# SamArgt/AudioSourceSep

Measured on AMD Instinct MI355X. Metric: Glow fwd+logdet passes/sec on 64×64×1 mel tiles (K=32,L=3), 1→8 MI355X, higher is better.
Workload: dtype f16x3

## Files before the change

audiosourcesep_amd/csrc/glowk.hip:

```cpp
#include "glowk_engine.h"
#include "glowk_light.h"

namespace glowk_eng {
thread_local std::string g_err;
}
using namespace glowk_eng;

namespace glowk_eng {

}

namespace glowk_detail {
int num_cus() {
  static int n = 0;
  if (n == 0) {
    int dev = 0; hipDeviceProp_t prop;
    if (hipGetDevice(&dev) == hipSuccess && hipGetDeviceProperties(&prop, dev) == hipSuccess) n = prop.multiProcessorCount;
    if (n <= 0) n = 256;
  }
  return n;
}
void launch_fail(const std::string& m) { fail(m); }
static EnvSwitches read_env() {
  auto on = [](const char* n) { return getenv(n) != nullptr; };
  return EnvSwitches{on("GLOWK_BWD_LIGHT_4"), on("GLOWK_NO_FUSE"), on("GLOWK_WGRAD_PLAIN"), on("GLOWK_CO_OFF"), on("GLOWK_Q_OFF"), on("GLOWK_CO_TRAIN_OFF"),
                     on("GLOWK_TRAIN_RECOMPUTE"), on("GLOWK_TRAIN_PERSTEP"), on("GLOWK_PG_JOIN")};
}
static EnvSwitches g_env = read_env();
const EnvSwitches& env() { return g_env; }
void reload_env() { g_env = read_env(); }
#define GLOWK_EXTERN_NET(CI_, NF_) extern template NetLaunch launch_net_t<CI_, NF_>(const NetArgs&, NetCall, hipStream_t, bool);
GLOWK_NET_SHAPES(GLOWK_EXTERN_NET)
#undef GLOWK_EXTERN_NET
}

namespace glowk_eng {
using glowk_detail::num_cus;
using glowk_detail::launch_net_t;

NetCall net_call(const glowk_handle* h, int dir, bool store, bool split) {
  if (h->precision == GLOWK_PREC_F32 || !split) return NetCall{dir, NET_EXACT, store};
  return NetCall{dir, h->precision == GLOWK_PREC_F16X2 && dir == NET_FWD && !store ? NET_SPLIT2 : NET_SPLIT3, store};
}

int* flagp(const glowk_handle* h) { return h->precision == GLOWK_PREC_F32 ? nullptr : h->d_flag; }

float bwd_norm_target(float xlim_b) {
  if (!(xlim_b >= 0.125f)) return 0.0f;
  int e = 0;
  std::frexp(xlim_b * 0.5f, &e);
  return std::ldexp(1.0f, std::min(e - 1, 10));
}

NetLaunch launch_net_raw(int c, int F, const NetArgs& a, NetCall call, hipStream_t s, bool dry) {
#define NETCASE(CI_, NF_) if (c == 2 * CI_ && F == 32 * NF_) return launch_net_t<CI_, NF_>(a, call, s, dry);
  GLOWK_NET_SHAPES(NETCASE)
#undef NETCASE
  return glowk_detail::net_failed("unsupported (channels, n_filters) combination: c=" + std::to_string(c) + " F=" + std::to_string(F));
}

int launch_net(glowk_handle* h, int level, int c, int F, const NetArgs& a, hipStream_t s, NetCall call, NetLaunch* out = nullptr) {
  if (h->profiling) {
    while (h->ev_pool.size() < h->ev_used + 2) {
      OwnedEvent e;
      HIPCHK(event_create(e, hipEventDefault));
      h->ev_pool.push_back(std::move(e));
    }
    HIPCHK(hipEventRecord(h->ev_pool[h->ev_used], s));
  }
  const NetLaunch r = launch_net_raw(c, F, a, call, s);
  if (!r.failed) {
    ++h->family_launches[r.family];
    if (r.co) ++h->family_launches[FAM_CO];
    if (r.q) ++h->family_launches[FAM_Q];
  }
  if (h->profiling) {
    HIPCHK(hipEventRecord(h->ev_pool[h->ev_used + 1], s));
    h->ev_used += 2;
// ... 1143 lines not shown
```

audiosourcesep_amd/csrc/glowk_co.h:

```cpp
#pragma once
#include "glowk_kernels.h"

constexpr int CO_PX = 128;
constexpr int CO_PSTR = 132;

template <int KIN, int MOUT, int NF, int MODE>
struct RingC {
  static constexpr int MODE7 = net_dir<MODE>;
  using S = RingS<KIN, MOUT, NF, MODE7, 2>;
  static constexpr bool FUSE = (MODE & NET_FUSE) != 0;
  static constexpr bool SAVE = MODE7 == NET_FWD_SAVE, BWD = MODE7 == NET_BWD;
  static constexpr bool MERGE = S::NMT <= 3;
  static constexpr bool M0LAST = S::NMT % 3 == 2;
  static constexpr bool STORE = (MODE & NET_STORE) != 0;
  static constexpr int MODEX = net_dir<MODE> | (MODE & NET_STORE);
  static constexpr int NFH = S::NFH, NRB = S::NRB, NMT = S::NMT, KS = S::KS;
  static constexpr int UNITP = S::MAINP / 2;
  static constexpr int UNIT4 = S::MAIN4 / 2;
  static constexpr int PPW = UNITP / 4;
  static constexpr int NG = NFH / 2;
  static constexpr int K1PW = (S::K1P + 3) / 4;
  static constexpr int EPN = BWD ? 0 : S::EPN;
  static constexpr int MASKN = BWD ? 2 * 4 * NF * 64 : 0;
  static constexpr size_t LDS_BYTES = (size_t)3 * UNIT4 * 16 + (size_t)2 * S::K14 * 16 + (size_t)EPN * 4 + (size_t)MASKN * 2 +
                                      (FUSE ? (size_t)36 * CO_PSTR * 4 + CO_PX * 16 : 0);
  static constexpr bool FITS = (MODE7 == NET_FWD || MODE7 == NET_FWD2 || SAVE || BWD) && !(MODE & NET_HALF) && (!STORE || ((SAVE || BWD) && !FUSE)) && S::NGRP == 1 && (NMT == 2 || NMT == 3 || (NMT == 5 && !STORE && !BWD)) &&
                               (!FUSE || (MOUT == 36 && !BWD)) && KS <= 3 && NF % 4 == 0 && NFH >= 2 && NFH % 2 == 0 && UNITP % 4 == 0 && PPW == NG &&
                               2 * LDS_BYTES <= 160 * 1024 + 1;
  static constexpr int XST = STORE ? 8 : 0;
  static constexpr int z_acts(int z) { int n = 0; for (int t = z * NFH; t < (z + 1) * NFH; ++t) n += (t % NMT == 0) ? 1 : 0; return n; }
  static constexpr int z_st(int z) { return STORE ? z_acts(z) * (8 + (SAVE ? 1 : 0)) : 0; }
  __device__ static const float4* main_unit(const float4* img, int pass, int i, int half) { return S::main_chunk(img, pass, i) + (size_t)half * UNIT4; }
  __device__ static const float4* out_unit(const float4* img, int pass, int z) { return S::out_chunk(img, pass, 0) + (size_t)z * UNIT4; }
};

__device__ __forceinline__ void co_bar() {
  __builtin_amdgcn_s_waitcnt(0xC07F);
  h3_barrier();
}

template <int N>
__device__ __forceinline__ void co_end() {
  __builtin_amdgcn_s_waitcnt((N & 15) | 0x0070 | ((N >> 4) << 14));
  h3_barrier();
}
template <int N>
__device__ __forceinline__ void co_end_st(bool more) {
  if (more) co_end<N + 1>();
  else co_end<N>();
}

struct CoCtx {
  float4 *m0, *m1, *d;
  const float4* img;
  int w4;
  unsigned voff;
};

template <int NFH, int MODE7, int H, int TAG, int K1P>
__device__ __forceinline__ void co_Y(const float4* slot, const h8 (&bh)[2], const h8 (&bl)[2], f32x4 (&acc2)[2 * NFH][2], int lane,
                                     const float4* src, float4* dst, int w4, unsigned voff) {
  const h8* buf = reinterpret_cast<const h8*>(slot) + lane;
  const char* ub = uniform_ptr(src);
  constexpr int NG = NFH / 2;
  h8 A[2][4];
  auto load = [&](h8 (&d)[4], int gi) {
    d[0] = buf[((2 * gi) * 2 + 0) * 64];
    d[1] = buf[((2 * gi) * 2 + 1) * 64];
    d[2] = buf[((2 * gi + 1) * 2 + 0) * 64];
    d[3] = buf[((2 * gi + 1) * 2 + 1) * 64];
  };
  load(A[0], 0);
#pragma unroll
  for (int gi = 0; gi < NG; ++gi) {
    const int o0 = H * NFH + 2 * gi, o1 = o0 + 1;
    if (gi + 1 < NG) load(A[(gi + 1) & 1], gi + 1);
    if constexpr (H == 1) {
      const int piece = gi * 4 + w4;
// ... 102 lines not shown
}

template <int KIN, int MOUT, int NF, int MODE, int PASS, bool SOLO>
__device__ __forceinline__ void co_pass(const NetArgs& a, const H3Ctx& hc, const CoCtx& c, const float* epl, float* pl,
                                        const h8 (&xh)[(RingC<KIN, MOUT, NF, MODE>::KS)][2], const h8 (&xl)[(RingC<KIN, MOUT, NF, MODE>::KS)][2],
                                        const int (&q)[2], const bool (&qok)[2], int lane, int kq, f32x4 (&keep)[(RingC<KIN, MOUT, NF, MODE>::NMT)][2]) {
  using G = RingC<KIN, MOUT, NF, MODE>;
  using S = typename G::S;
  constexpr int NRB = G::NRB, NFH = G::NFH, MODE7 = G::MODE7;
  constexpr int f2base = PASS * NFH * 32;
  constexpr bool SECOND = !SOLO && PASS == 1;
  f32x4 acc2[NRB][2];
#pragma unroll
  for (int ob = 0; ob < NRB; ++ob)
#pragma unroll
    for (int r = 0; r < 4; ++r) {
      const float b = G::BWD ? 0.0f : epl[f2base + ob * 16 + 4 * kq + r];
      acc2[ob][0][r] = b;
      acc2[ob][1][r] = b;
    }
  const bool st = G::SAVE && PASS == 0 && hc.wok;
  constexpr int XST = PASS == 0 ? G::XST : 0;
  h8 bh[2], bl[2];
#pragma nounroll
  for (int i0 = 0; i0 < NF; i0 += 2) {
    if (i0 > 0 || (SECOND && !G::M0LAST)) stage4<G::UNITP, 73>(G::main_unit(c.img, PASS, i0, 1), c.m1, c.w4, c.voff);
    if constexpr (SECOND && G::M0LAST) {
      if (i0 == 0) stage4<G::UNITP, 77>(G::main_unit(c.img, PASS, 0, 0), c.m0, c.w4, c.voff);
    }
    h3s_X<KIN, MOUT, NF, G::MODEX, 2, 0, PASS, G::STORE>(a, hc, i0, xh, xl, lane, bh, bl);
    if (SECOND && G::M0LAST && i0 == 0) co_end<0>();
    else co_end_st<G::PPW + XST>(st);
    co_Y<NFH, MODE7, 0, 1, S::K1P>(c.m0, bh, bl, acc2, lane, hc.k1img + (size_t)((i0 + 2) % NF) * S::K14, hc.k1s0, c.w4, c.voff);
    co_end_st<G::K1PW + XST>(st);
    co_Y<NFH, MODE7, 1, 2, S::K1P>(c.m1, bh, bl, acc2, lane, G::main_unit(c.img, PASS, i0 + 1, 0), c.m0, c.w4, c.voff);
    co_bar();
    stage4<G::UNITP, 74>(G::main_unit(c.img, PASS, i0 + 1, 1), c.m1, c.w4, c.voff);
    h3s_X<KIN, MOUT, NF, G::MODEX, 2, 1, PASS, G::STORE>(a, hc, i0 + 1, xh, xl, lane, bh, bl);
    co_end_st<G::PPW + XST>(st);
    co_Y<NFH, MODE7, 0, 3, S::K1P>(c.m0, bh, bl, acc2, lane, hc.k1img + (size_t)((i0 + 3) % NF) * S::K14, hc.k1s1, c.w4, c.voff);
    co_end_st<G::K1PW + XST>(st);
    co_Y<NFH, MODE7, 1, 4, S::K1P>(c.m1, bh, bl, acc2, lane, i0 + 2 < NF ? G::main_unit(c.img, PASS, i0 + 2, 0) : G::out_unit(c.img, PASS, 1), c.m0,
                                   c.w4, c.voff);
    co_bar();
  }
  f32x4 acc3[G::NMT][2];
  co_Z<KIN, MOUT, NF, MODE, PASS, SOLO, 0>(a, hc, c, epl, pl, acc2, acc3, bh, bl, q, qok, lane, kq, keep);
  co_Z<KIN, MOUT, NF, MODE, PASS, SOLO, 1>(a, hc, c, epl, pl, acc2, acc3, bh, bl, q, qok, lane, kq, keep);
  if constexpr (G::NMT >= 3) co_Z<KIN, MOUT, NF, MODE, PASS, SOLO, 2>(a, hc, c, epl, pl, acc2, acc3, bh, bl, q, qok, lane, kq, keep);
  if constexpr (G::NMT >= 4) co_Z<KIN, MOUT, NF, MODE, PASS, SOLO, 3>(a, hc, c, epl, pl, acc2, acc3, bh, bl, q, qok, lane, kq, keep);
  if constexpr (G::NMT >= 5) co_Z<KIN, MOUT, NF, MODE, PASS, SOLO, 4>(a, hc, c, epl, pl, acc2, acc3, bh, bl, q, qok, lane, kq, keep);
}

template <int KIN, int MOUT, int NF, int MODE, bool SPLIT>
__global__ __launch_bounds__(256, 2) void k_net_h3c(NetArgs a) {
  using G = RingC<KIN, MOUT, NF, MODE>;
  using S = typename G::S;
  constexpr int KS = G::KS;
  constexpr int SGN = G::BWD ? -1 : 1;
  static_assert(G::FITS, "shape");
  static_assert(!(G::FUSE && SPLIT), "the fused coupling needs both passes in one workgroup");

  const int tid = threadIdx.x;
  __shared__ __attribute__((aligned(1024))) float4 slotM0[G::UNIT4];
  __shared__ __attribute__((aligned(1024))) float4 slotM1[G::UNIT4];
  __shared__ __attribute__((aligned(1024))) float4 slotD[G::UNIT4];
  __shared__ __attribute__((aligned(1024))) float4 k1slot0[S::K14];
  __shared__ __attribute__((aligned(1024))) float4 k1slot1[S::K14];
  float* epl = nullptr;
  if constexpr (!G::BWD) { __shared__ float epl_arr[S::EPN]; epl = epl_arr; }
  unsigned short* mkl = nullptr;
  if constexpr (G::BWD) { __shared__ __attribute__((aligned(1024))) unsigned short mkl_arr[G::MASKN]; mkl = mkl_arr; }
  float* plds = nullptr;
  float4* vstash = nullptr;
  if constexpr (G::FUSE) {
    __shared__ float plds_arr[36 * CO_PSTR];
    __shared__ float4 vstash_arr[CO_PX];
    plds = plds_arr; vstash = vstash_arr;
  }
  const int lane = tid & 63;
  const int wave = __builtin_amdgcn_readfirstlane(tid >> 6);
  const int n16 = lane & 15;
  const int kq = lane >> 4;
  const int qbase = ((int)blockIdx.x * 4 + wave) * 32;
  const int q[2] = {G::STORE ? qbase + 2 * n16 : qbase + n16, G::STORE ? qbase + 2 * n16 + 1 : qbase + 16 + n16};
  const bool qok[2] = {q[0] < a.Q, q[1] < a.Q};
  const int pass0 = SPLIT ? (int)blockIdx.y : 0;

  H3Ctx hc;
  hc.sA = hc.sB = hc.sD = nullptr; hc.k1s0 = k1slot0; hc.k1s1 = k1slot1;
  hc.k1img = a.RSp; hc.img = a.RSp; hc.mkl = mkl; hc.mk2off = 4 * NF * 64; hc.pl = plds;
  hc.wblk = (size_t)blockIdx.x * 4 + wave;
  hc.wok = (long)hc.wblk * 32 < a.Q;
  hc.w4 = wave; hc.voff = (unsigned)lane * 16u; hc.ub[0] = hc.ub[1] = 1.0f;
  CoCtx c;
  c.m0 = slotM0; c.m1 = slotM1; c.d = slotD; c.img = a.RSp; c.w4 = wave; c.voff = (unsigned)lane * 16u;

  stage4<G::UNITP, 60>(G::main_unit(c.img, pass0, 0, 0), slotM0, c.w4, c.voff);
  stage4<G::UNITP, 61>(G::main_unit(c.img, pass0, 0, 1), slotM1, c.w4, c.voff);
  stage4<G::UNITP, 62>(G::out_unit(c.img, pass0, 0), slotD, c.w4, c.voff);
  stage4<S::K1P, 63>(hc.k1img, k1slot0, c.w4, c.voff);
  stage4<S::K1P, 64>(hc.k1img + S::K14, k1slot1, c.w4, c.voff);
  if constexpr (G::BWD) {
    stage4<NF / 2, 65>(reinterpret_cast<const float4*>(a.mask1 + (size_t)blockIdx.x * 4 * NF * 64), reinterpret_cast<float4*>(mkl), c.w4, c.voff);
    stage4<NF / 2, 66>(reinterpret_cast<const float4*>(a.mask2 + (size_t)blockIdx.x * 4 * NF * 64), reinterpret_cast<float4*>(mkl + 4 * NF * 64), c.w4, c.voff);
  }

  h8 xh[KS][2], xl[KS][2];
  float xmax = 0.0f;
  {
    const int hw = a.h * a.w;
#pragma unroll
    for (int hf = 0; hf < 2; ++hf) {
      const int qq = qok[hf] ? q[hf] : 0;
      const int rem = qq % hw;
      const int i = rem / a.w, j0 = rem % a.w;
      const float* base = a.vin + (long)qq * a.in_stride + a.in_off;
      if constexpr (G::BWD) {
        float v[KS][8];
        float pm = 0.0f;
#pragma unroll
        for (int s = 0; s < KS; ++s) {
          gather8<KIN, false, SGN>(base, i, j0, a.h, a.w, a.in_stride, qok[hf], 32 * s + 8 * kq, v[s]);
          pm = range8(pm, v[s]);
        }
        pm = nan_max(pm, __shfl_xor(pm, 16, 64));
        pm = nan_max(pm, __shfl_xor(pm, 32, 64));
        xmax = nan_max(xmax, pm);
        const float fac = G::STORE ? 1.0f : pixel_norm(pm, a.bnorm, hc.ub[hf]);
#pragma unroll
        for (int s = 0; s < KS; ++s) {
#pragma unroll
          for (int j = 0; j < 8; ++j) v[s][j] *= fac;
          split8(v[s], xh[s][hf], xl[s][hf]);
        }
      } else if constexpr (S::STK) {
        xmax = gather_stacked<KIN, SGN, G::MODE7 == NET_FWD2, KS, S::KSX>(base, i, j0, a.h, a.w, a.in_stride, qok[hf], kq, xh, xl, hf, xmax);
      } else {
#pragma unroll
        for (int s = 0; s < KS; ++s) {
          float v[8];
          gather8<KIN, true, SGN>(base, i, j0, a.h, a.w, a.in_stride, qok[hf], 32 * s + 8 * kq, v);
          xmax = range8(xmax, v);
          split8(v, xh[s][hf], xl[s][hf]);
        }
      }
    }
  }
  if constexpr (G::FUSE) {
    if (tid < CO_PX) {
      const int qv = (int)blockIdx.x * CO_PX + tid;
      vstash[tid] = qv < a.Q ? *reinterpret_cast<const float4*>(a.vin + (size_t)qv * 4) : float4{0.f, 0.f, 0.f, 0.f};
    }
  }
  if constexpr (!G::BWD)
    for (int i = tid; i < S::EPN; i += 256) epl[i] = a.eph[i];
  if (((G::BWD && !G::STORE) ? !(xmax <= 3.0e38f) : !(xmax <= a.xlim)) && a.flag) *a.flag = 1;
  if (a.xmax_out) range_probe(a.xmax_out, xmax);
  asm volatile("s_waitcnt vmcnt(0)" ::: "memory");
  __syncthreads();

  f32x4 keep[G::NMT][2];
  if constexpr (SPLIT) {
    if (pass0 == 0) co_pass<KIN, MOUT, NF, MODE, 0, true>(a, hc, c, epl, plds, xh, xl, q, qok, lane, kq, keep);
    else co_pass<KIN, MOUT, NF, MODE, 1, true>(a, hc, c, epl, plds, xh, xl, q, qok, lane, kq, keep);
  } else {
    co_pass<KIN, MOUT, NF, MODE, 0, false>(a, hc, c, epl, plds, xh, xl, q, qok, lane, kq, keep);
    co_pass<KIN, MOUT, NF, MODE, 1, false>(a, hc, c, epl, plds, xh, xl, q, qok, lane, kq, keep);
  }
  if constexpr (G::FUSE) {
    __syncthreads();
    fused_couple<CO_PX, CO_PSTR>(a, plds, vstash, tid);
  }
}
```

audiosourcesep_amd/csrc/glowk_kernels.h:

```cpp
#pragma once
#include "glowk_act_scale.h"

#include <hip/hip_runtime.h>
#include <utility>
#include <stdint.h>

typedef float f32x16 __attribute__((ext_vector_type(16)));

#define GLOWK_GPTR(p) ((const __attribute__((address_space(1))) void*)(p))
#define GLOWK_LPTR(p) ((__attribute__((address_space(3))) void*)(p))

__device__ __forceinline__ int mfma_row(int r, int hh) { return (r & 3) + 8 * (r >> 2) + 4 * hh; }

struct NetArgs {
  const float* vin;
  int in_stride, in_off;
  int Q, h, w;
  const float* K1p;
  const float* ep;
  const float4* R0p;
  unsigned short* mask1;
  unsigned short* mask2;
  float* P;
  size_t pstride;
// ... 1186 lines not shown
                                         f32x4 (&acc3)[(RingS<KIN, MOUT, NF, MODE, NP>::G0N)][2], h8 (&bh)[2], h8 (&bl)[2], int g, const int (&q)[2],
                                         const bool (&qok)[2], int lane, int kq, f32x4 (&keep)[(RingS<KIN, MOUT, NF, MODE, NP>::G0N)][2],
                                         std::integer_sequence<int, Z...>) {
  (h3s_Z<KIN, MOUT, NF, MODE, NP, P0, PASS, SOLO, Z>(a, c, epl, acc2, acc3, bh, bl, g, q, qok, lane, kq, keep), ...);
}

template <int KIN, int MOUT, int NF, int MODE, int NP, int P0, int PASS, bool SOLO>
__device__ __forceinline__ void h3s_pass(const NetArgs& a, const H3Ctx& c, const float* epl, const h8 (&xh)[(RingS<KIN, MOUT, NF, MODE, NP>::KS)][2],
                                         const h8 (&xl)[(RingS<KIN, MOUT, NF, MODE, NP>::KS)][2], int g, const int (&q)[2], const bool (&qok)[2], int lane, int kq,
                                         f32x4 (&keep)[(RingS<KIN, MOUT, NF, MODE, NP>::G0N)][2]) {
  using G = RingS<KIN, MOUT, NF, MODE, NP>;
  constexpr int NRB = G::NRB;
  constexpr int f2base = PASS * G::NFH * 32;
  f32x4 acc2[NRB][2];
#pragma unroll
  for (int ob = 0; ob < NRB; ++ob)
#pragma unroll
    for (int r = 0; r < 4; ++r) {
      const float b = net_dir<MODE> == NET_BWD ? 0.0f : epl[f2base + ob * 16 + 4 * kq + r];
      acc2[ob][0][r] = b;
      acc2[ob][1][r] = b;
    }
  h8 bh[2], bl[2];
#pragma nounroll
  for (int i0 = 0; i0 < NF; i0 += 2) {
    h3s_X<KIN, MOUT, NF, MODE, NP, 0, PASS>(a, c, i0, xh, xl, lane, bh, bl);
    h3_x_end<MODE, PASS, 8 * G::PXH>(c);
    if (PASS >= 1 && !SOLO && G::NCH == 1 && i0 == 0 && !g)
      stage4<G::MAINP, 50>(G::out_chunk(c.img, PASS, 0), c.sD, c.w4, c.voff);
    h3s_Y<KIN, MOUT, NF, MODE, NP, 1>(P0 ? c.sB : c.sA, bh, bl, acc2, lane, g, true, G::main_chunk(c.img, PASS, i0 + 1), P0 ? c.sA : c.sB,
                         c.k1img + (size_t)((i0 + 2) % NF) * G::K14, c.k1s0, c.w4, c.voff);
    h3_barrier();
    h3s_X<KIN, MOUT, NF, MODE, NP, 1, PASS>(a, c, i0 + 1, xh, xl, lane, bh, bl);
    h3_x_end<MODE, PASS, 8 * G::PXH>(c);
    h3s_Y<KIN, MOUT, NF, MODE, NP, 2>(P0 ? c.sA : c.sB, bh, bl, acc2, lane, g, i0 + 2 < NF || G::NCH >= 2,
                         i0 + 2 < NF ? G::main_chunk(c.img, PASS, i0 + 2) : G::out_chunk(c.img, PASS, 1),
                         P0 ? c.sB : c.sA, c.k1img + (size_t)((i0 + 3) % NF) * G::K14, c.k1s1, c.w4, c.voff);
    h3_barrier();
  }
  f32x4 acc3[G::G0N][2];
  h3s_tail<KIN, MOUT, NF, MODE, NP, P0, PASS, SOLO>(a, c, epl, acc2, acc3, bh, bl, g, q, qok, lane, kq, keep, std::make_integer_sequence<int, 2 * G::NCH>());
}

template <int KIN, int MOUT, int NF, int MODE, int NP, int PASS, int P0>
__device__ __forceinline__ void h3s_passes(const NetArgs& a, const H3Ctx& c, const float* epl, const h8 (&xh)[(RingS<KIN, MOUT, NF, MODE, NP>::KS)][2],
                                           const h8 (&xl)[(RingS<KIN, MOUT, NF, MODE, NP>::KS)][2], int g, const int (&q)[2], const bool (&qok)[2], int lane, int kq,
                                           f32x4 (&keep)[(RingS<KIN, MOUT, NF, MODE, NP>::G0N)][2]) {
  h3s_pass<KIN, MOUT, NF, MODE, NP, P0, PASS, false>(a, c, epl, xh, xl, g, q, qok, lane, kq, keep);
  if constexpr (PASS + 1 < NP) h3s_passes<KIN, MOUT, NF, MODE, NP, PASS + 1, (RingS<KIN, MOUT, NF, MODE, NP>::NCH + 1 + P0) & 1>(a, c, epl, xh, xl, g, q, qok, lane, kq, keep);
}

__device__ __forceinline__ bool fz_not_finite(float v) { return !(fabsf(v) <= 3.0e38f); }

template <int PXW = 256, int PSTR = FUSE_PSTR>
__device__ __forceinline__ void fused_couple(const NetArgs& a, const float* pl, const float4* vst, int tid) {
  const int wave = tid >> 6, lane = tid & 63;
  const int px = wave * 32 + (lane & 31), k = lane >> 5;
  const int q = (int)blockIdx.x * PXW + px;
  const bool qok = q < a.Q;
  const int w = a.w, hw = a.h * a.w, nrows = PXW / w;
  const int pp = (qok ? q : 0) % hw;
  const int i = pp / w, j = pp % w, r = px / w;
  float ols = 0.0f, ot = 0.0f;
  bool missing = false;
#pragma unroll
  for (int tap = 0; tap < 9; ++tap) {
    const int dy = tap / 3 - 1, dx = tap % 3 - 1;
    const int ii = i + dy, jj = j + dx;
    if (ii < 0 || ii >= a.h || jj < 0 || jj >= w) continue;
    const int rr = r + dy;
    if (rr < 0 || rr >= nrows) { missing = true; continue; }
    const int spx = px + dy * w + dx;
    ols += pl[(tap * 4 + k) * PSTR + spx];
    ot += pl[(tap * 4 + 2 + k) * PSTR + spx];
  }
  ols += a.fz_b3[k];
  ot += a.fz_b3[2 + k];
  float lsum = 0.0f;
  const float4 v4 = vst[px];
  const float vk = k ? v4.y : v4.x;
  const float log_s = tanhf(ols);
  const float sc = expf(log_s);
  const float yk = a.fz_inverse ? (vk - ot) / sc : sc * vk + ot;
  const float yo = __shfl_xor(yk, 32, 64);
  const float y[4] = {k ? yo : yk, k ? yk : yo, v4.z, v4.w};
  if (qok && a.fz_osave) a.fz_osave[(size_t)q * 2 + k] = ols;
  if (qok && !missing) {
    lsum = log_s;
    bool bad = fz_not_finite(ols) | fz_not_finite(ot) | fz_not_finite(yk);
    if (bad && a.flag) *a.flag = 1;
    float z0, z1;
    if (a.fz_A) {
      z0 = a.fz_b[2 * k]; z1 = a.fz_b[2 * k + 1];
#pragma unroll
      for (int ci = 0; ci < 4; ++ci) {
        z0 = fmaf(y[ci], a.fz_A[ci * 4 + 2 * k], z0);
        z1 = fmaf(y[ci], a.fz_A[ci * 4 + 2 * k + 1], z1);
      }
    } else {
      z0 = y[2 * k]; z1 = y[2 * k + 1];
    }
    *reinterpret_cast<float2*>(a.fz_out + (size_t)q * a.fz_out_stride + a.fz_out_off + 2 * k) = float2{z0, z1};
  } else if (qok) {
    float* e = a.fz_edge + (((size_t)blockIdx.x * 4 + (r == 0 ? 0 : 1)) * FUSE_EW + j) * 4;
    e[k] = ols;
    e[2 + k] = ot;
  }
  for (int te = tid; te < 2 * w * 4; te += 2 * PXW) {
    const int which = te / (4 * w), jt = (te / 4) % w, ch = te & 3;
    float hsum = 0.0f;
#pragma unroll
    for (int dx = -1; dx <= 1; ++dx) {
      const int js = jt + dx;
      if (js < 0 || js >= w) continue;
      const int tap = (which ? 0 : 6) + dx + 1;
      hsum += pl[(tap * 4 + ch) * PSTR + (which ? (nrows - 1) * w : 0) + js];
    }
    a.fz_edge[(((size_t)blockIdx.x * 4 + 2 + which) * FUSE_EW + jt) * 4 + ch] = hsum;
  }
  if (a.fz_ldpart) {
    double d = (double)lsum;
#pragma unroll
    for (int o = 32; o > 0; o >>= 1) d += __shfl_down(d, o, 64);
    if (lane == 0) a.fz_ldpart[(size_t)blockIdx.x * (PXW / 32) + wave] = d;
  }
}

template <int KIN, int MOUT, int NF, int MODE, int NP, bool SPLIT>
__global__ __launch_bounds__(512, 2) void k_net_h3s(NetArgs a) {
  using G = RingS<KIN, MOUT, NF, MODE, NP>;
  constexpr int KS = G::KS;
  constexpr int SGN = (net_dir<MODE> == NET_BWD) ? -1 : 1;
  static_assert(G::FITS, "shape");

  __shared__ float4 slotA[G::MAIN4];
  __shared__ float4 slotB[G::MAIN4];
  __shared__ float4 slotD[G::MAIN4];
  __shared__ float4 k1slot0[G::K14];
  __shared__ float4 k1slot1[G::K14];
  __shared__ float epl[G::EPN];
  __shared__ __attribute__((aligned(16))) unsigned short mkl[G::MASK2B / 2 + 8];
  __shared__ float plds[G::FUSE ? 36 * FUSE_PSTR : 1];
  __shared__ float4 vstash[G::FUSE ? 256 : 1];
  static_assert(!G::FUSE || (G::MERGE && !SPLIT && MOUT == 36), "the fused coupling needs both passes in one workgroup and a 4-channel level");
  static_assert(!(MODE & NET_STORE) || G::PXH == 1, "hidden stores (training): half-wave form only -- with two pixel halves a wave whose second half lies "
                                            "beyond Q would issue fewer stores than h3_x_end's counted wait assumes");

  const int tid = threadIdx.x;
  const int lane = tid & 63;
  const int wave = __builtin_amdgcn_readfirstlane(tid >> 6);
  const int g = wave >> 2;
  const int n16 = lane & 15;
  const int kq = lane >> 4;
  const int qbase = (blockIdx.x * 8 + (tid >> 6)) * (16 * G::PXH);
  const int q[2] = {qbase + n16, G::PXH == 2 ? qbase + 16 + n16 : qbase + n16};
  const bool qok[2] = {q[0] < a.Q, G::PXH == 2 && q[1] < a.Q};

  H3Ctx c;
  c.sA = slotA; c.sB = slotB; c.sD = slotD; c.k1s0 = k1slot0; c.k1s1 = k1slot1;
  const int solo_pass = SPLIT ? (int)blockIdx.y : 0;
  c.k1img = a.RSp;
  c.img = a.RSp;
  c.mkl = mkl;
  c.mk2off = 8 * NF * 64;
  c.pl = plds;
  c.wblk = (size_t)blockIdx.x * 8 + wave;
  c.wok = (long)c.wblk * (16 * G::PXH) < a.Q;
  c.w4 = wave & 3;
  c.voff = (unsigned)lane * 16u;
  c.ub[0] = c.ub[1] = 1.0f;

  if (!g) {
    stage4<G::MAINP, 60>(G::main_chunk(c.img, solo_pass, 0), slotA, c.w4, c.voff);
    stage4<G::MAINP, 61>(G::out_chunk(c.img, solo_pass, 0), slotD, c.w4, c.voff);
    if (net_dir<MODE> == NET_BWD)
      stage4<NF, 64>(reinterpret_cast<const float4*>(a.mask1 + (size_t)blockIdx.x * 8 * NF * 64), reinterpret_cast<float4*>(mkl), c.w4, c.voff);
  } else {
    stage4<G::K1P, 62>(c.k1img, k1slot0, c.w4, c.voff);
// ... 78 lines not shown
```

audiosourcesep_amd/csrc/glowk_launch.h:

```cpp
#pragma once
#include "glowk_kernels.h"
#include "glowk_co.h"
#include "glowk_q.h"

#include <cstdlib>
#include <string>

#define GLOWK_NET_SHAPES(X) X(2, 16) X(4, 16) X(8, 16) X(16, 16) X(2, 12) X(4, 12) X(8, 12) X(16, 12) \
                            X(2, 8) X(4, 8) X(8, 8) X(16, 8) X(2, 4) X(4, 4) X(8, 4) X(16, 4)

enum NetArith { NET_EXACT, NET_SPLIT3, NET_SPLIT2 };
struct NetCall { int dir; NetArith arith; bool store = false; };

enum NetFamily { FAM_F32, FAM_H3, FAM_H3S, FAM_H3S_HALF, FAM_FUSED, FAM_CO, FAM_Q, FAM_COUNT };

struct NetLaunch {
  int np = 0;
  int family = FAM_F32;
  bool co = false;
  bool q = false;
  int fused_px = 0;
  bool failed = false;
  explicit operator bool() const { return np > 0 || fused_px > 0; }
};

namespace glowk_detail {

int num_cus();
void launch_fail(const std::string&);

struct EnvSwitches {
  bool bwd_light_4;
  bool no_fuse;
  bool wgrad_plain;
  bool co_off;
  bool q_off;
  bool co_train_off;
  bool train_recompute;
  bool train_perstep;
  bool pg_join;
};
const EnvSwitches& env();

template <int CI, int DIR>
struct NetShape {
  static constexpr int KIN = DIR == NET_BWD ? 2 * CI : CI;
  static constexpr int MOUT = DIR == NET_BWD ? 9 * CI : 18 * CI;
};

template <int CI, int NF, int DIR, bool STORE>
NetLaunch launch_f32(const NetArgs& a, hipStream_t s, bool dry) {
  using Sh = NetShape<CI, DIR>;
  if (!dry) hipLaunchKernelGGL((k_net_f32<Sh::KIN, Sh::MOUT, NF, DIR, STORE>), dim3((a.Q + 127) / 128), dim3(256), 0, s, a);
  return {1, FAM_F32};
}

template <int KIN, int MOUT, int NF, int MODE>
NetLaunch launch_h3(const NetArgs& a, hipStream_t s, bool dry) {
  constexpr bool F2 = RingH<KIN, MOUT, NF, MODE, 2>::FITS, F4 = RingH<KIN, MOUT, NF, MODE, 4>::FITS;
  const int wgs = (a.Q + 255) / 256, cus = num_cus();
  if constexpr (F4) {
    if (a.max_np >= 4 && (4 * wgs <= cus || !F2)) {
      const bool split = 4 * wgs <= cus;
      if (!dry) {
        if (split) hipLaunchKernelGGL((k_net_h3<KIN, MOUT, NF, MODE, 4, true>), dim3(wgs, 4), dim3(512), 0, s, a);
        else hipLaunchKernelGGL((k_net_h3<KIN, MOUT, NF, MODE, 4, false>), dim3(wgs), dim3(512), 0, s, a);
      }
      return {4, FAM_H3};
    }
  }
  if constexpr (F2) {
    if (!dry) {
      if (2 * wgs <= cus) hipLaunchKernelGGL((k_net_h3<KIN, MOUT, NF, MODE, 2, true>), dim3(wgs, 2), dim3(512), 0, s, a);
      else hipLaunchKernelGGL((k_net_h3<KIN, MOUT, NF, MODE, 2, false>), dim3(wgs), dim3(512), 0, s, a);
    }
    return {2, FAM_H3};
  }
  return {};
}

template <class Kernel>
inline bool co_two_per_cu(Kernel kernel) {
  static int blocks = -1;
  if (blocks < 0) {
    int n = 0;
    if (hipOccupancyMaxActiveBlocksPerMultiprocessor(&n, kernel, 256, 0) != hipSuccess) { (void)hipGetLastError(); n = 0; }
    blocks = n;
  }
  return blocks >= 2;
}

template <int KIN, int MOUT, int NF, int MODE>
NetLaunch launch_h3s(const NetArgs& a, hipStream_t s, bool dry) {
  static_assert(!(MODE & NET_STORE), "no storing launches here: the co-resident branch does not check Q % 128 (launch_co_train does)");
  constexpr bool F2 = RingS<KIN, MOUT, NF, MODE, 2>::FITS, F4 = RingS<KIN, MOUT, NF, MODE, 4>::FITS;
  const int wgs = (a.Q + 255) / 256, cus = num_cus();
  if constexpr (F4) {
    if (a.max_np >= 4 && (4 * wgs <= cus || !F2)) {
      const bool split = 4 * wgs <= cus;
      if (!dry) {
        if (split) hipLaunchKernelGGL((k_net_h3s<KIN, MOUT, NF, MODE, 4, true>), dim3(wgs, 4), dim3(512), 0, s, a);
        else hipLaunchKernelGGL((k_net_h3s<KIN, MOUT, NF, MODE, 4, false>), dim3(wgs), dim3(512), 0, s, a);
      }
      return {4, FAM_H3S};
    }
  }
  if constexpr (F2) {
    const bool split = 2 * wgs <= cus;
    if constexpr (RingC<KIN, MOUT, NF, MODE>::FITS) {
      const int wgc = (a.Q + CO_PX - 1) / CO_PX;
      const bool co_ok = a.co && !env().co_off;
      if (co_ok && wgc > cus) {
        if constexpr (RingC<KIN, MOUT, NF, MODE | NET_FUSE>::FITS) {
          if (a.fuse && co_two_per_cu(k_net_h3c<KIN, MOUT, NF, MODE | NET_FUSE, false>)) {
            if (!dry) hipLaunchKernelGGL((k_net_h3c<KIN, MOUT, NF, MODE | NET_FUSE, false>), dim3(wgc), dim3(256), 0, s, a);
            return {0, FAM_FUSED, true, false, CO_PX};
          }
        }
        if (!a.fuse && co_two_per_cu(k_net_h3c<KIN, MOUT, NF, MODE, false>)) {
          if (!dry) hipLaunchKernelGGL((k_net_h3c<KIN, MOUT, NF, MODE, false>), dim3(wgc), dim3(256), 0, s, a);
          return {RingC<KIN, MOUT, NF, MODE>::MERGE ? 1 : 2, FAM_H3S, true};
        }
      }
      if (co_ok && split && wgc <= cus && a.max_np >= 2 && co_two_per_cu(k_net_h3c<KIN, MOUT, NF, MODE, true>)) {
        if (!dry) hipLaunchKernelGGL((k_net_h3c<KIN, MOUT, NF, MODE, true>), dim3(wgc, 2), dim3(256), 0, s, a);
        return {2, FAM_H3S, true};
      }
    }
    if constexpr ((MODE == NET_FWD || MODE == NET_FWD2 || MODE == NET_FWD_SAVE) && MOUT == 36) {
      if constexpr (RingS<KIN, MOUT, NF, MODE | NET_FUSE, 2>::FITS && RingS<KIN, MOUT, NF, MODE | NET_FUSE, 2>::MERGE) {
        if (a.fuse && !split) {
          if (!dry) hipLaunchKernelGGL((k_net_h3s<KIN, MOUT, NF, MODE | NET_FUSE, 2, false>), dim3(wgs), dim3(512), 0, s, a);
          return {0, FAM_FUSED, false, false, 256};
        }
      }
    }
    if (!dry) {
      if (split) hipLaunchKernelGGL((k_net_h3s<KIN, MOUT, NF, MODE, 2, true>), dim3(wgs, 2), dim3(512), 0, s, a);
      else hipLaunchKernelGGL((k_net_h3s<KIN, MOUT, NF, MODE, 2, false>), dim3(wgs), dim3(512), 0, s, a);
    }
    return {(!split && RingS<KIN, MOUT, NF, MODE, 2>::MERGE) ? 1 : 2, FAM_H3S};
  }
  return {};
}

inline bool half_wave_grid(const NetArgs& a) { return 8 * ((a.Q + 255) / 256) <= num_cus(); }

template <int KIN, int MOUT, int NF, int MODE>
NetLaunch launch_h3s_half(const NetArgs& a, hipStream_t s, bool dry) {
  if constexpr (RingS<KIN, MOUT, NF, MODE | NET_HALF, 4>::FITS) {
    if (a.max_np < 4) return {};
    const int wgs = (a.Q + 127) / 128;
    if constexpr (RingQ<KIN, MOUT, NF, MODE>::FITS) {
      if (4 * wgs <= num_cus() && !env().q_off) {
        if (!dry) hipLaunchKernelGGL((k_net_h3q<KIN, MOUT, NF, MODE>), dim3(wgs, 4), dim3(512), 0, s, a);
        return {4, FAM_H3S_HALF, false, true};
      }
    }
    if (!dry) {
      if (4 * wgs <= num_cus()) hipLaunchKernelGGL((k_net_h3s<KIN, MOUT, NF, MODE | NET_HALF, 4, true>), dim3(wgs, 4), dim3(512), 0, s, a);
      else hipLaunchKernelGGL((k_net_h3s<KIN, MOUT, NF, MODE | NET_HALF, 4, false>), dim3(wgs), dim3(512), 0, s, a);
    }
    return {4, FAM_H3S_HALF};
  }
  return {};
}
// ... 139 lines not shown
```

Baseline: 15920.

## Double-buffer the fused coupling conv ring with four LDS slots

Adds a four-slot double-buffered LDS ring for the fused forward coupling kernel (MOUT=36). Each half-step's MFMA work overlaps the DMA of the next unit into the alternate slot pair, which removes the per-step barrier stalls of the three-slot ring. The coupling partial sums reuse the ring slots in place of a separate plds buffer, and fused_couple now takes three tile pointers. The old three-slot path stays reachable through GLOWK_CO_RING3. The risk is higher LDS use, which could threaten two workgroups per CU, and more complex synchronisation.

```diff
diff --git a/audiosourcesep_amd/csrc/glowk.hip b/audiosourcesep_amd/csrc/glowk.hip
--- a/audiosourcesep_amd/csrc/glowk.hip
+++ b/audiosourcesep_amd/csrc/glowk.hip
@@ -23,7 +23,7 @@
 void launch_fail(const std::string& m) { fail(m); }
 static EnvSwitches read_env() {
   auto on = [](const char* n) { return getenv(n) != nullptr; };
-  return EnvSwitches{on("GLOWK_BWD_LIGHT_4"), on("GLOWK_NO_FUSE"), on("GLOWK_WGRAD_PLAIN"), on("GLOWK_CO_OFF"), on("GLOWK_Q_OFF"), on("GLOWK_CO_TRAIN_OFF"),
+  return EnvSwitches{on("GLOWK_BWD_LIGHT_4"), on("GLOWK_NO_FUSE"), on("GLOWK_WGRAD_PLAIN"), on("GLOWK_CO_OFF"), on("GLOWK_CO_RING3"), on("GLOWK_Q_OFF"), on("GLOWK_CO_TRAIN_OFF"),
                      on("GLOWK_TRAIN_RECOMPUTE"), on("GLOWK_TRAIN_PERSTEP"), on("GLOWK_PG_JOIN")};
 }
 static EnvSwitches g_env = read_env();
diff --git a/audiosourcesep_amd/csrc/glowk_co.h b/audiosourcesep_amd/csrc/glowk_co.h
--- a/audiosourcesep_amd/csrc/glowk_co.h
+++ b/audiosourcesep_amd/csrc/glowk_co.h
@@ -24,6 +24,10 @@
   static constexpr int MASKN = BWD ? 2 * 4 * NF * 64 : 0;
   static constexpr size_t LDS_BYTES = (size_t)3 * UNIT4 * 16 + (size_t)2 * S::K14 * 16 + (size_t)EPN * 4 + (size_t)MASKN * 2 +
                                       (FUSE ? (size_t)36 * CO_PSTR * 4 + CO_PX * 16 : 0);
+  static constexpr bool DB = FUSE && (MODE7 == NET_FWD || MODE7 == NET_FWD2) && MOUT == 36;
+  static constexpr int PTILE4 = (16 * CO_PSTR * 4 + 1023) / 1024 * 64;
+  static constexpr int DBSLOT4 = UNIT4 > PTILE4 ? UNIT4 : PTILE4;
+  static constexpr size_t LDS_BYTES_DB = (size_t)4 * DBSLOT4 * 16 + (size_t)2 * S::K14 * 16 + (size_t)EPN * 4 + CO_PX * 16;
   static constexpr bool FITS = (MODE7 == NET_FWD || MODE7 == NET_FWD2 || SAVE || BWD) && !(MODE & NET_HALF) && (!STORE || ((SAVE || BWD) && !FUSE)) && S::NGRP == 1 && (NMT == 2 || NMT == 3 || (NMT == 5 && !STORE && !BWD)) &&
                                (!FUSE || (MOUT == 36 && !BWD)) && KS <= 3 && NF % 4 == 0 && NFH >= 2 && NFH % 2 == 0 && UNITP % 4 == 0 && PPW == NG &&
                                2 * LDS_BYTES <= 160 * 1024 + 1;
@@ -232,7 +236,148 @@
   if constexpr (G::NMT >= 5) co_Z<KIN, MOUT, NF, MODE, PASS, SOLO, 4>(a, hc, c, epl, pl, acc2, acc3, bh, bl, q, qok, lane, kq, keep);
 }
 
-template <int KIN, int MOUT, int NF, int MODE, bool SPLIT>
+struct CoCtxDB {
+  float4 *s0, *s1, *s2, *s3;
+  const float4* img;
+  int w4;
+  unsigned voff;
+};
+
+template <int NFH, int MODE7, int TAG, int K1P>
+__device__ __forceinline__ void co_Ydb(const float4* sa, const float4* sb, const h8 (&bh)[2], const h8 (&bl)[2], f32x4 (&acc2)[2 * NFH][2], int lane,
+                                       const float4* srca, float4* dsta, const float4* srcb, float4* dstb, const float4* k1src, float4* k1dst,
+                                       int w4, unsigned voff) {
+  const h8* bufa = reinterpret_cast<const h8*>(sa) + lane;
+  const h8* bufb = reinterpret_cast<const h8*>(sb) + lane;
+  const char* uba = uniform_ptr(srca);
+  const char* ubb = uniform_ptr(srcb);
+  constexpr int NG = NFH / 2;
+  h8 A[2][4];
+  auto load = [&](h8 (&d)[4], int g) {
+    const h8* buf = g < NG ? bufa : bufb;
+    const int gi = g % NG;
+    d[0] = buf[((2 * gi) * 2 + 0) * 64];
+    d[1] = buf[((2 * gi) * 2 + 1) * 64];
+    d[2] = buf[((2 * gi + 1) * 2 + 0) * 64];
+    d[3] = buf[((2 * gi + 1) * 2 + 1) * 64];
+  };
+  load(A[0], 0);
+#pragma unroll
+  for (int g = 0; g < 2 * NG; ++g) {
+    const int gi = g % NG;
+    const int o0 = (g / NG) * NFH + 2 * gi, o1 = o0 + 1;
+    if (g + 1 < 2 * NG) load(A[(g + 1) & 1], g + 1);
+    const int piece = gi * 4 + w4;
+    if (g < NG) glds16(reinterpret_cast<const float4*>(uba + (size_t)piece * 1024 + voff), dsta + piece * 64);
+    else glds16(reinterpret_cast<const float4*>(ubb + (size_t)piece * 1024 + voff), dstb + piece * 64);
+    asm volatile("; dma site %0" ::"n"(TAG * 16 + g));
+    if (g == 0) stage4<K1P, TAG * 16 + 15>(k1src, k1dst, w4, voff);
+    __builtin_amdgcn_sched_barrier(0);
+    const h8 (&af)[4] = A[g & 1];
+    acc2[o0][0] = __builtin_amdgcn_mfma_f32_16x16x32_f16(af[1], bh[0], acc2[o0][0], 0, 0, 0);
+    acc2[o0][1] = __builtin_amdgcn_mfma_f32_16x16x32_f16(af[1], bh[1], acc2[o0][1], 0, 0, 0);
+    acc2[o1][0] = __builtin_amdgcn_mfma_f32_16x16x32_f16(af[3], bh[0], acc2[o1][0], 0, 0, 0);
+    acc2[o1][1] = __builtin_amdgcn_mfma_f32_16x16x32_f16(af[3], bh[1], acc2[o1][1], 0, 0, 0);
+    if (MODE7 != NET_FWD2) {
+      acc2[o0][0] = __builtin_amdgcn_mfma_f32_16x16x32_f16(af[0], bl[0], acc2[o0][0], 0, 0, 0);
+      acc2[o0][1] = __builtin_amdgcn_mfma_f32_16x16x32_f16(af[0], bl[1], acc2[o0][1], 0, 0, 0);
+      acc2[o1][0] = __builtin_amdgcn_mfma_f32_16x16x32_f16(af[2], bl[0], acc2[o1][0], 0, 0, 0);
+      acc2[o1][1] = __builtin_amdgcn_mfma_f32_16x16x32_f16(af[2], bl[1], acc2[o1][1], 0, 0, 0);
+    }
+    acc2[o0][0] = __builtin_amdgcn_mfma_f32_16x16x32_f16(af[0], bh[0], acc2[o0][0], 0, 0, 0);
+    acc2[o0][1] = __builtin_amdgcn_mfma_f32_16x16x32_f16(af[0], bh[1], acc2[o0][1], 0, 0, 0);
+    acc2[o1][0] = __builtin_amdgcn_mfma_f32_16x16x32_f16(af[2], bh[0], acc2[o1][0], 0, 0, 0);
+    acc2[o1][1] = __builtin_amdgcn_mfma_f32_16x16x32_f16(af[2], bh[1], acc2[o1][1], 0, 0, 0);
+    __builtin_amdgcn_sched_barrier(0);
+  }
+}
+
+template <int KIN, int MOUT, int NF, int MODE, int PASS, int Z>
+__device__ __forceinline__ void co_Zdb(const NetArgs& a, const CoCtxDB& c, const float* epl, f32x4 (&acc2)[(RingC<KIN, MOUT, NF, MODE>::NRB)][2],
+                                       f32x4 (&acc3)[3][2], h8 (&bh)[2], h8 (&bl)[2], int lane, int kq, f32x4 (&keep)[3][2]) {
+  using G = RingC<KIN, MOUT, NF, MODE>;
+  constexpr int NFH = G::NFH, NMT = G::NMT, M3 = MOUT, MODE7 = G::MODE7;
+  static_assert(NMT == 3 && G::MERGE && G::FUSE, "the double-buffered ring: three conv3 units, merged passes, fused coupling");
+  constexpr bool NEXT = PASS == 0;
+  if constexpr (Z == 0) stage4<G::UNITP, 90>(G::out_unit(c.img, PASS, 2), c.s2, c.w4, c.voff);
+  if constexpr (Z == 1 && NEXT) stage4<G::UNITP, 91>(G::main_unit(c.img, PASS + 1, 0, 0), c.s0, c.w4, c.voff);
+  if constexpr (Z == 2 && NEXT) stage4<G::UNITP, 92>(G::main_unit(c.img, PASS + 1, 0, 1), c.s1, c.w4, c.voff);
+  const float4* slot = Z == 0 ? c.s0 : Z == 1 ? c.s1 : c.s2;
+  const h8* buf = reinterpret_cast<const h8*>(slot) + lane;
+  const float* pb = epl + NF * 32;
+#pragma unroll
+  for (int tp = 0; tp < NFH; ++tp) {
+    const int t = Z * NFH + tp;
+    const int fo = t / NMT, ml = t % NMT;
+    if (ml == 0) {
+#pragma unroll
+      for (int hf = 0; hf < 2; ++hf) h3s_act<MODE7, false>(acc2[2 * fo][hf], acc2[2 * fo + 1][hf], a.sc2, 0u, bh[hf], bl[hf]);
+    }
+    if (fo == 0) {
+#pragma unroll
+      for (int r = 0; r < 4; ++r) { acc3[ml][0][r] = 0.0f; acc3[ml][1][r] = 0.0f; }
+    }
+    const h8 ah = buf[(tp * 2 + 0) * 64], al = buf[(tp * 2 + 1) * 64];
+    acc3[ml][0] = mfma3s<MODE7 == NET_FWD2>(ah, al, bh[0], bl[0], acc3[ml][0]);
+    acc3[ml][1] = mfma3s<MODE7 == NET_FWD2>(ah, al, bh[1], bl[1], acc3[ml][1]);
+    if (fo == NFH - 1) {
+      float* pt = reinterpret_cast<float*>(ml == 0 ? c.s0 : ml == 1 ? c.s1 : c.s3);
+#pragma unroll
+      for (int hf = 0; hf < 2; ++hf)
+#pragma unroll
+        for (int r = 0; r < 4; ++r) {
+          const int m = ml * 16 + 4 * kq + r;
+          const float part = PASS == 0 ? fmaf(acc3[ml][hf][r], a.sc3, pb[m]) : acc3[ml][hf][r] * a.sc3;
+          if constexpr (NEXT) { keep[ml][hf][r] = part; continue; }
+          const float val = part + keep[ml][hf][r];
+          if (m < M3) pt[(4 * kq + r) * CO_PSTR + (int)(threadIdx.x >> 6) * 32 + 16 * hf + (lane & 15)] = val;
+        }
+    }
+  }
+  if constexpr (Z == 0) co_bar();
+  if constexpr (Z == 1) co_end<(NEXT ? G::PPW : 0)>();
+  if constexpr (Z == 2 && NEXT) co_bar();
+}
+
+template <int KIN, int MOUT, int NF, int MODE, int PASS>
+__device__ __forceinline__ void co_pass_db(const NetArgs& a, const H3Ctx& hc, const CoCtxDB& c, const float* epl,
+                                           const h8 (&xh)[(RingC<KIN, MOUT, NF, MODE>::KS)][2], const h8 (&xl)[(RingC<KIN, MOUT, NF, MODE>::KS)][2],
+                                           int lane, int kq, f32x4 (&keep)[3][2]) {
+  using G = RingC<KIN, MOUT, NF, MODE>;
+  using S = typename G::S;
+  constexpr int NRB = G::NRB, NFH = G::NFH, MODE7 = G::MODE7;
+  constexpr int f2base = PASS * NFH * 32;
+  f32x4 acc2[NRB][2];
+#pragma unroll
+  for (int ob = 0; ob < NRB; ++ob)
+#pragma unroll
+    for (int r = 0; r < 4; ++r) {
+      const float b = epl[f2base + ob * 16 + 4 * kq + r];
+      acc2[ob][0][r] = b;
+      acc2[ob][1][r] = b;
+    }
+  h8 bh[2], bl[2];
+#pragma nounroll
+  for (int i0 = 0; i0 < NF; i0 += 2) {
+    h3s_X<KIN, MOUT, NF, G::MODEX, 2, 0, PASS, false>(a, hc, i0, xh, xl, lane, bh, bl);
+    co_end<0>();
+    co_Ydb<NFH, MODE7, 1, S::K1P>(c.s0, c.s1, bh, bl, acc2, lane, G::main_unit(c.img, PASS, i0 + 1, 0), c.s2, G::main_unit(c.img, PASS, i0 + 1, 1), c.s3,
+                                  hc.k1img + (size_t)((i0 + 2) % NF) * S::K14, hc.k1s0, c.w4, c.voff);
+    h3s_X<KIN, MOUT, NF, G::MODEX, 2, 1, PASS, false>(a, hc, i0 + 1, xh, xl, lane, bh, bl);
+    co_end<0>();
+    const bool more = i0 + 2 < NF;
+    co_Ydb<NFH, MODE7, 2, S::K1P>(c.s2, c.s3, bh, bl, acc2, lane, more ? G::main_unit(c.img, PASS, i0 + 2, 0) : G::out_unit(c.img, PASS, 0), c.s0,
+                                  more ? G::main_unit(c.img, PASS, i0 + 2, 1) : G::out_unit(c.img, PASS, 1), c.s1,
+                                  hc.k1img + (size_t)((i0 + 3) % NF) * S::K14, hc.k1s1, c.w4, c.voff);
+  }
+  co_end<0>();
+  f32x4 acc3[3][2];
+  co_Zdb<KIN, MOUT, NF, MODE, PASS, 0>(a, c, epl, acc2, acc3, bh, bl, lane, kq, keep);
+  co_Zdb<KIN, MOUT, NF, MODE, PASS, 1>(a, c, epl, acc2, acc3, bh, bl, lane, kq, keep);
+  co_Zdb<KIN, MOUT, NF, MODE, PASS, 2>(a, c, epl, acc2, acc3, bh, bl, lane, kq, keep);
+}
+
+template <int KIN, int MOUT, int NF, int MODE, bool SPLIT, bool RING3 = false>
 __global__ __launch_bounds__(256, 2) void k_net_h3c(NetArgs a) {
   using G = RingC<KIN, MOUT, NF, MODE>;
   using S = typename G::S;
@@ -240,11 +385,25 @@
   constexpr int SGN = G::BWD ? -1 : 1;
   static_assert(G::FITS, "shape");
   static_assert(!(G::FUSE && SPLIT), "the fused coupling needs both passes in one workgroup");
+  constexpr bool DB = G::DB && !SPLIT && !RING3;
+  static_assert(!RING3 || G::DB, "RING3 names the three-slot form of an instance that has both");
+  static_assert(!DB || 2 * G::LDS_BYTES_DB <= 160 * 1024, "two workgroups per CU");
 
   const int tid = threadIdx.x;
-  __shared__ __attribute__((aligned(1024))) float4 slotM0[G::UNIT4];
-  __shared__ __attribute__((aligned(1024))) float4 slotM1[G::UNIT4];
-  __shared__ __attribute__((aligned(1024))) float4 slotD[G::UNIT4];
+  CoCtx c;
+  CoCtxDB cd;
+  if constexpr (DB) {
+    __shared__ __attribute__((aligned(1024))) float4 slotS0[G::DBSLOT4];
+    __shared__ __attribute__((aligned(1024))) float4 slotS1[G::DBSLOT4];
+    __shared__ __attribute__((aligned(1024))) float4 slotS2[G::DBSLOT4];
+    __shared__ __attribute__((aligned(1024))) float4 slotS3[G::DBSLOT4];
+    cd.s0 = slotS0; cd.s1 = slotS1; cd.s2 = slotS2; cd.s3 = slotS3;
+  } else {
+    __shared__ __attribute__((aligned(1024))) float4 slotM0[G::UNIT4];
+    __shared__ __attribute__((aligned(1024))) float4 slotM1[G::UNIT4];
+    __shared__ __attribute__((aligned(1024))) float4 slotD[G::UNIT4];
+    c.m0 = slotM0; c.m1 = slotM1; c.d = slotD;
+  }
   __shared__ __attribute__((aligned(1024))) float4 k1slot0[S::K14];
   __shared__ __attribute__((aligned(1024))) float4 k1slot1[S::K14];
   float* epl = nullptr;
@@ -253,11 +412,8 @@
   if constexpr (G::BWD) { __shared__ __attribute__((aligned(1024))) unsigned short mkl_arr[G::MASKN]; mkl = mkl_arr; }
   float* plds = nullptr;
   float4* vstash = nullptr;
-  if constexpr (G::FUSE) {
-    __shared__ float plds_arr[36 * CO_PSTR];
-    __shared__ float4 vstash_arr[CO_PX];
-    plds = plds_arr; vstash = vstash_arr;
-  }
+  if constexpr (G::FUSE && !DB) { __shared__ float plds_arr[36 * CO_PSTR]; plds = plds_arr; }
+  if constexpr (G::FUSE) { __shared__ float4 vstash_arr[CO_PX]; vstash = vstash_arr; }
   const int lane = tid & 63;
   const int wave = __builtin_amdgcn_readfirstlane(tid >> 6);
   const int n16 = lane & 15;
@@ -273,12 +429,17 @@
   hc.wblk = (size_t)blockIdx.x * 4 + wave;
   hc.wok = (long)hc.wblk * 32 < a.Q;
   hc.w4 = wave; hc.voff = (unsigned)lane * 16u; hc.ub[0] = hc.ub[1] = 1.0f;
-  CoCtx c;
-  c.m0 = slotM0; c.m1 = slotM1; c.d = slotD; c.img = a.RSp; c.w4 = wave; c.voff = (unsigned)lane * 16u;
-
-  stage4<G::UNITP, 60>(G::main_unit(c.img, pass0, 0, 0), slotM0, c.w4, c.voff);
-  stage4<G::UNITP, 61>(G::main_unit(c.img, pass0, 0, 1), slotM1, c.w4, c.voff);
-  stage4<G::UNITP, 62>(G::out_unit(c.img, pass0, 0), slotD, c.w4, c.voff);
+  c.img = a.RSp; c.w4 = wave; c.voff = (unsigned)lane * 16u;
+  cd.img = a.RSp; cd.w4 = wave; cd.voff = (unsigned)lane * 16u;
+
+  if constexpr (DB) {
+    stage4<G::UNITP, 58>(G::main_unit(cd.img, 0, 0, 0), cd.s0, c.w4, c.voff);
+    stage4<G::UNITP, 59>(G::main_unit(cd.img, 0, 0, 1), cd.s1, c.w4, c.voff);
+  } else {
+    stage4<G::UNITP, 60>(G::main_unit(c.img, pass0, 0, 0), c.m0, c.w4, c.voff);
+    stage4<G::UNITP, 61>(G::main_unit(c.img, pass0, 0, 1), c.m1, c.w4, c.voff);
+    stage4<G::UNITP, 62>(G::out_unit(c.img, pass0, 0), c.d, c.w4, c.voff);
+  }
   stage4<S::K1P, 63>(hc.k1img, k1slot0, c.w4, c.voff);
   stage4<S::K1P, 64>(hc.k1img + S::K14, k1slot1, c.w4, c.voff);
   if constexpr (G::BWD) {
@@ -341,14 +502,19 @@
   __syncthreads();
 
   f32x4 keep[G::NMT][2];
-  if constexpr (SPLIT) {
+  if constexpr (DB) {
+    co_pass_db<KIN, MOUT, NF, MODE, 0>(a, hc, cd, epl, xh, xl, lane, kq, keep);
+    co_pass_db<KIN, MOUT, NF, MODE, 1>(a, hc, cd, epl, xh, xl, lane, kq, keep);
+    __syncthreads();
+    fused_couple<CO_PX, CO_PSTR>(a, reinterpret_cast<const float*>(cd.s0), reinterpret_cast<const float*>(cd.s1), reinterpret_cast<const float*>(cd.s3), vstash, tid);
+  } else if constexpr (SPLIT) {
     if (pass0 == 0) co_pass<KIN, MOUT, NF, MODE, 0, true>(a, hc, c, epl, plds, xh, xl, q, qok, lane, kq, keep);
     else co_pass<KIN, MOUT, NF, MODE, 1, true>(a, hc, c, epl, plds, xh, xl, q, qok, lane, kq, keep);
   } else {
     co_pass<KIN, MOUT, NF, MODE, 0, false>(a, hc, c, epl, plds, xh, xl, q, qok, lane, kq, keep);
     co_pass<KIN, MOUT, NF, MODE, 1, false>(a, hc, c, epl, plds, xh, xl, q, qok, lane, kq, keep);
   }
-  if constexpr (G::FUSE) {
+  if constexpr (G::FUSE && !DB) {
     __syncthreads();
     fused_couple<CO_PX, CO_PSTR>(a, plds, vstash, tid);
   }
diff --git a/audiosourcesep_amd/csrc/glowk_kernels.h b/audiosourcesep_amd/csrc/glowk_kernels.h
--- a/audiosourcesep_amd/csrc/glowk_kernels.h
+++ b/audiosourcesep_amd/csrc/glowk_kernels.h
@@ -1262,8 +1262,9 @@
 
 __device__ __forceinline__ bool fz_not_finite(float v) { return !(fabsf(v) <= 3.0e38f); }
 
+__device__ __forceinline__ const float* fz_tile(const float* pl0, const float* pl1, const float* pl2, int tile) { return tile == 0 ? pl0 : tile == 1 ? pl1 : pl2; }
 template <int PXW = 256, int PSTR = FUSE_PSTR>
-__device__ __forceinline__ void fused_couple(const NetArgs& a, const float* pl, const float4* vst, int tid) {
+__device__ __forceinline__ void fused_couple(const NetArgs& a, const float* pl0, const float* pl1, const float* pl2, const float4* vst, int tid) {
   const int wave = tid >> 6, lane = tid & 63;
   const int px = wave * 32 + (lane & 31), k = lane >> 5;
   const int q = (int)blockIdx.x * PXW + px;
@@ -1281,8 +1282,9 @@
     const int rr = r + dy;
     if (rr < 0 || rr >= nrows) { missing = true; continue; }
     const int spx = px + dy * w + dx;
-    ols += pl[(tap * 4 + k) * PSTR + spx];
-    ot += pl[(tap * 4 + 2 + k) * PSTR + spx];
+    const float* pt = fz_tile(pl0, pl1, pl2, tap / 4) + (tap % 4) * 4 * PSTR;
+    ols += pt[k * PSTR + spx];
+    ot += pt[(2 + k) * PSTR + spx];
   }
   ols += a.fz_b3[k];
   ot += a.fz_b3[2 + k];
@@ -1324,7 +1326,7 @@
       const int js = jt + dx;
       if (js < 0 || js >= w) continue;
       const int tap = (which ? 0 : 6) + dx + 1;
-      hsum += pl[(tap * 4 + ch) * PSTR + (which ? (nrows - 1) * w : 0) + js];
+      hsum += fz_tile(pl0, pl1, pl2, tap / 4)[((tap % 4) * 4 + ch) * PSTR + (which ? (nrows - 1) * w : 0) + js];
     }
     a.fz_edge[(((size_t)blockIdx.x * 4 + 2 + which) * FUSE_EW + jt) * 4 + ch] = hsum;
   }
@@ -1334,6 +1336,11 @@
     for (int o = 32; o > 0; o >>= 1) d += __shfl_down(d, o, 64);
     if (lane == 0) a.fz_ldpart[(size_t)blockIdx.x * (PXW / 32) + wave] = d;
   }
+}
+
+template <int PXW = 256, int PSTR = FUSE_PSTR>
+__device__ __forceinline__ void fused_couple(const NetArgs& a, const float* pl, const float4* vst, int tid) {
+  fused_couple<PXW, PSTR>(a, pl, pl + 16 * PSTR, pl + 32 * PSTR, vst, tid);
 }
 
 template <int KIN, int MOUT, int NF, int MODE, int NP, bool SPLIT>
diff --git a/audiosourcesep_amd/csrc/glowk_launch.h b/audiosourcesep_amd/csrc/glowk_launch.h
--- a/audiosourcesep_amd/csrc/glowk_launch.h
+++ b/audiosourcesep_amd/csrc/glowk_launch.h
@@ -34,6 +34,7 @@
   bool no_fuse;
   bool wgrad_plain;
   bool co_off;
+  bool co_ring3;
   bool q_off;
   bool co_train_off;
   bool train_recompute;
@@ -112,6 +113,12 @@
       const bool co_ok = a.co && !env().co_off;
       if (co_ok && wgc > cus) {
         if constexpr (RingC<KIN, MOUT, NF, MODE | NET_FUSE>::FITS) {
+          if constexpr (RingC<KIN, MOUT, NF, MODE | NET_FUSE>::DB) {
+            if (a.fuse && env().co_ring3 && co_two_per_cu(k_net_h3c<KIN, MOUT, NF, MODE | NET_FUSE, false, true>)) {
+              if (!dry) hipLaunchKernelGGL((k_net_h3c<KIN, MOUT, NF, MODE | NET_FUSE, false, true>), dim3(wgc), dim3(256), 0, s, a);
+              return {0, FAM_FUSED, true, false, CO_PX};
+            }
+          }
           if (a.fuse && co_two_per_cu(k_net_h3c<KIN, MOUT, NF, MODE | NET_FUSE, false>)) {
             if (!dry) hipLaunchKernelGGL((k_net_h3c<KIN, MOUT, NF, MODE | NET_FUSE, false>), dim3(wgc), dim3(256), 0, s, a);
             return {0, FAM_FUSED, true, false, CO_PX};
```

Result: faster. 16090, median of 6 (+1.0%).
